# NVIDIA/cuopt

Measured on AMD Instinct MI355X. Metric: pdlp_iterations_per_sec, higher is better.
Workload: dtype f64; 1 GPU; c3: synthetic random sparse LP S(m=1000000,n=1000000,k=10,seed=2), nnz=10000000, longest row 10, CSR fp64/int32, Stable2 preset, tolerances 0 (fixed iteration budget); rows=1000000, cols=1000000, nnz=10000000, parallelism=single GPU

## Files before the change

### cuopt_amd/csrc/pdlp_epilogues.hpp

```cpp
#pragma once
#include "pdlp_kernels.hpp"

using namespace pdlp;

namespace p2pdev {
struct Peers {
  char* base[16];
};
constexpr int kKinds = 3;
__device__ __forceinline__ bool active(const pdlpdev_ctl* ctl) { return ctl->error == 0 && ctl->steps_taken < ctl->target_steps; }

struct Push {
  Peers P;
  int world, rank, kind;
  size_t dst_off, flag_off;
  unsigned long long* epoch;
  int lo[16], hi[16];
  __device__ __forceinline__ double* slot(int q) const { return reinterpret_cast<double*>(P.base[q] + dst_off); }
  __device__ __forceinline__ bool wants(int q, int i) const { return q != rank && i >= lo[q] && i < hi[q]; }
};
__device__ __forceinline__ void put(double* p, double v) { __hip_atomic_store(p, v, __ATOMIC_RELAXED, __HIP_MEMORY_SCOPE_SYSTEM); }
__device__ __forceinline__ void count_exchange(const Push* T)
{
  if (blockIdx.x == 0 && threadIdx.x == 0) T->epoch[T->kind] = T->epoch[T->kind] + 1;
}
__device__ __forceinline__ void raise(const Push* T)
{
  if (blockIdx.x != 0 || threadIdx.x != 0) return;
  const unsigned long long e = T->epoch[T->kind];
  for (int q = 0; q < T->world; ++q) {
    unsigned long long* flag = reinterpret_cast<unsigned long long*>(T->P.base[q] + T->flag_off) + (size_t)T->kind * T->world + T->rank;
    __hip_atomic_store(flag, e, __ATOMIC_RELEASE, __HIP_MEMORY_SCOPE_SYSTEM);
  }
}
__device__ __forceinline__ bool wait_flags(const unsigned long long* flags, int world, int kind, const unsigned long long* epoch)
{
  bool ok = true;
  if ((int)threadIdx.x < world) {
    const unsigned long long want = epoch[kind];
    const unsigned long long* f   = flags + (size_t)kind * world + threadIdx.x;
    const unsigned long long t0   = wall_clock64();
    while (__hip_atomic_load(f, __ATOMIC_RELAXED, __HIP_MEMORY_SCOPE_SYSTEM) < want) {
      __builtin_amdgcn_s_sleep(8);
      if (wall_clock64() - t0 > 500000000ull) {
        ok = false;
        break;
      }
    }
  }
  ok = __syncthreads_and(ok);
  if (threadIdx.x == 0) __threadfence_system();
  __syncthreads();
  return ok;
}
}


struct DualEpilogue {
  static constexpr int NQ = 1;
  using Op = SumOp;
  const double* __restrict__ y;
  double* __restrict__ yn;
  const double* __restrict__ lo;
  const double* __restrict__ hi;
  double* __restrict__ sumy;
  double sigma, weight;
  bool pend;
  double* __restrict__ copy = nullptr;
  const p2pdev::Push* __restrict__ push = nullptr;
  struct Ops {
    double y, lo, hi, sum;
  };
  __device__ __forceinline__ Ops load(int i) const { return Ops{y[i], lo[i], hi[i], pend ? sumy[i] : 0.0}; }
  __device__ __forceinline__ void apply(int i, double v, const Ops& o, double (&acc)[1])
  {
    const double yi = o.y;
    double next     = yi - (sigma * v);
    const double low = next + sigma * o.lo;
    const double up  = next + sigma * o.hi;
    next            = dmax(low, dmin(up, 0.0));
    yn[i]           = next;
    if (copy) copy[i] = next;
    if (push)
      for (int q = 0; q < push->world; ++q)
        if (push->wants(q, i)) p2pdev::put(push->slot(q) + i, next);
    const double dy = next - yi;
    acc[0] += dy * dy;
    if (pend) sumy[i] = o.sum + weight * yi;
  }
  __device__ __forceinline__ void row(int i, double v, double (&acc)[1]) { apply(i, v, load(i), acc); }
  static __device__ __forceinline__ DualEpilogue make(const pdlpdev_ctl* ctl, double* y0, double* y1, const double* lo, const double* hi,
                                                      double* sumy, double* ycopy, const p2pdev::Push* push)
  {
    const int cur = ctl->cur;
    return DualEpilogue{cur ? y1 : y0, cur ? y0 : y1, lo, hi, sumy, ctl->sigma, ctl->step_size, ctl->pending_avg != 0, ycopy, push};
  }
};

struct StepEpilogue {
  static constexpr int NQ = 2;
  using Op = SumOp;
  const double* __restrict__ x;
  const double* __restrict__ xn;
  const double* __restrict__ aty;
  double* __restrict__ atyn;
  struct Ops {
    double x, xn, aty;
  };
  __device__ __forceinline__ Ops load(int j) const { return Ops{x[j], xn[j], aty[j]}; }
  __device__ __forceinline__ void apply(int j, double v, const Ops& o, double (&acc)[2])
  {
    atyn[j]         = v;
    const double dx = o.xn - o.x;
    const double t  = v - o.aty;
    acc[0] += t * dx;
    acc[1] += dx * dx;
  }
  __device__ __forceinline__ void row(int j, double v, double (&acc)[2]) { apply(j, v, load(j), acc); }
  static __device__ __forceinline__ StepEpilogue make(const pdlpdev_ctl* ctl, const double* x0, const double* x1, double* aty0, double* aty1)
  {
    const int cur = ctl->cur;
    return StepEpilogue{cur ? x1 : x0, cur ? x0 : x1, cur ? aty1 : aty0, cur ? aty0 : aty1};
  }
};

struct HalpernWeights {
  double w, w0;
  __device__ __forceinline__ explicit HalpernWeights(const pdlpdev_halpern* hal)
  {
    const double k = (double)hal->k;
    w              = (k + 1.0) / (k + 2.0);
    w0             = 1.0 - w;
  }
  __device__ __forceinline__ double combine(double t, double z, double z0) const { return w * (2.0 * t - z) + w0 * z0; }
};
struct HalpernArgs {
  const pdlpdev_halpern* __restrict__ hal;
  double* __restrict__ tx;
  double* __restrict__ ty;
  const double* __restrict__ x0;
  const double* __restrict__ y0;
  const double* __restrict__ aty0;
};
__device__ __forceinline__ bool halpern_last_step(const pdlpdev_ctl* ctl) { return ctl->steps_taken + 1 >= ctl->target_steps; }
struct HalpernDualEpilogue {
  static constexpr int NQ = 1;
  using Op = SumOp;
  const double* __restrict__ y;
  double* __restrict__ yn;
  double* __restrict__ yp;
  const double* __restrict__ y0;
  const double* __restrict__ lo;
  const double* __restrict__ hi;
  double sigma;
  HalpernWeights hw;
  __device__ __forceinline__ void row(int i, double v, double (&acc)[1])
  {
    const double yi  = y[i];
    double next      = yi - (sigma * v);
    const double low = next + sigma * lo[i];
    const double up  = next + sigma * hi[i];
    next             = dmax(low, dmin(up, 0.0));
    yp[i]            = next;
    const double dy  = next - yi;
    acc[0] += dy * dy;
    yn[i] = hw.combine(next, yi, y0[i]);
  }
  static __device__ __forceinline__ HalpernDualEpilogue make(const pdlpdev_ctl* ctl, double* y0, double* y1, const double* lo, const double* hi,
                                                             const HalpernArgs& h)
  {
    const int cur = ctl->cur;
    return HalpernDualEpilogue{cur ? y1 : y0, cur ? y0 : y1, h.ty, h.y0, lo, hi, ctl->sigma, HalpernWeights(h.hal)};
  }
};
struct HalpernStepEpilogue {
  static constexpr int NQ = 2;
  using Op = SumOp;
  const double* __restrict__ x;
  double* __restrict__ xn;
  const double* __restrict__ aty;
  double* __restrict__ atyn;
  const double* __restrict__ x0;
  const double* __restrict__ aty0;
  double* __restrict__ xp;
  HalpernWeights hw;
  __device__ __forceinline__ void row(int j, double v, double (&acc)[2])
  {
    const double xj = x[j], xt = xn[j], a = aty[j];
    const double dx = xt - xj;
    const double t  = v - a;
    acc[0] += t * dx;
    acc[1] += dx * dx;
    if (xp) xp[j] = xt;
    xn[j]   = hw.combine(xt, xj, x0[j]);
    atyn[j] = hw.combine(v, a, aty0[j]);
  }
  static __device__ __forceinline__ HalpernStepEpilogue make(const pdlpdev_ctl* ctl, double* x0, double* x1, double* aty0, double* aty1,
                                                             const HalpernArgs& h)
  {
    const int cur = ctl->cur;
    return HalpernStepEpilogue{cur ? x1 : x0, cur ? x0 : x1, cur ? aty1 : aty0, cur ? aty0 : aty1, h.x0, h.aty0,
                               halpern_last_step(ctl) ? h.tx : nullptr, HalpernWeights(h.hal)};
  }
};

struct StoreEpilogue {
  static constexpr int NQ = 0;
  using Op = SumOp;
  double* __restrict__ out;
  __device__ __forceinline__ void row(int r, double v, double (&)[1]) { out[r] = v; }
  static __device__ __forceinline__ StoreEpilogue iterate(int side, double* aty0, double* aty1, double* out_override)
  {
    return StoreEpilogue{out_override ? out_override : (side ? aty1 : aty0)};
  }
};

__device__ __forceinline__ const double* evaluated(int cur, int which, const double* v0, const double* v1, const double* avg)
{
  return which == PDLPDEV_AVERAGE ? avg : (cur ? v1 : v0);
}

struct EvalPrimalEpilogue {
  static constexpr int NQ = 3;
  using Op = SumOp;
  const double* __restrict__ yhat;
  const double* __restrict__ dr;
  const double* __restrict__ lo_u;
  const double* __restrict__ hi_u;
  double eps_rel;
  double* __restrict__ linf_rows;
  double* __restrict__ ax_out;
  __device__ __forceinline__ void row(int i, double v, double (&acc)[3])
  {
    const double d  = dr[i];
    const double ax = v / d;
    ax_out[i]       = ax;
    const double yi = yhat[i] * d;
    const double lo = lo_u[i], hi = hi_u[i];
    const double rp = violation(ax, lo, hi);
    acc[0] += rp * rp;
    acc[1] += bound_value_product(yi, lo, hi);
    acc[2] += yi * yi;
    if (linf_rows) linf_rows[i] = rp - eps_rel * combine_bounds(lo, hi);
  }
};

struct EvalDualCore {
  const double* __restrict__ xhat;
  const double* __restrict__ dc;
  const double* __restrict__ c_u;
  const double* __restrict__ lb_u;
  const double* __restrict__ ub_u;
  double eps_rel;
  int rule_finite;
  double* __restrict__ rc_out;
  double* __restrict__ linf_rows;
  double* __restrict__ aty_out;
  __device__ __forceinline__ void col(int j, double aty_scaled, double (&acc)[4])
  {
    const double d    = dc[j];
    const double aty  = aty_scaled / d;
    aty_out[j]        = aty;
    const double cj   = c_u[j];
    const double g    = cj - aty;
    const double xj   = xhat[j] * d;
    const double lb   = lb_u[j], ub = ub_u[j];
    const double bv   = g > 0.0 ? lb : ub;
    double rc;
    if (g == 0.0)
      rc = g;
    else if (rule_finite)
      rc = dfinite(bv) ? g : 0.0;
    else
      rc = fabs(xj - bv) <= fabs(xj) ? g : 0.0;
    const double rd = g - rc;
    rc_out[j]       = rc;
    acc[0] += rd * rd;
    acc[1] += bound_value_product(rc, lb, ub);
    acc[2] += cj * xj;
    acc[3] += xj * xj;
    if (linf_rows) linf_rows[j] = rd - eps_rel * cj;
  }
};

struct EvalDualEpilogue {
  static constexpr int NQ = 4;
  using Op = SumOp;
  EvalDualCore core;
  __device__ __forceinline__ void row(int j, double v, double (&acc)[4]) { core.col(j, v, acc); }
};

struct DenseView {
  const int32_t* __restrict__ row;
  const int32_t* __restrict__ row_seg;
  const int32_t* __restrict__ seg_row;
  const int32_t* __restrict__ seg_c0;
  const int32_t* __restrict__ seg_len;
  const int32_t* __restrict__ seg_ptr;
  const int32_t* __restrict__ tile_ptr;
  const int32_t* __restrict__ tile_seg;
  const int32_t* __restrict__ tile_id;
  const double* __restrict__ val;
  const int32_t* __restrict__ ch_seg;
  const int32_t* __restrict__ ch_k0;
  const int32_t* __restrict__ row_ch;
  double* __restrict__ ch_part;
};

constexpr int kDenseChunk = 4096;

enum GatherMode : int {
  kGatherFixed   = 0,
  kGatherTrial   = 1,
  kGatherCurrent = 2,
};
static_assert(kGatherFixed == 0 && kGatherTrial == 1 && kGatherCurrent == 2, "the values of the kernels' `mode` argument");
__device__ __forceinline__ const double* pick_vector(const pdlpdev_ctl* ctl, const double* v0, const double* v1, int mode)
{
  if (mode == kGatherFixed) return v0;
  const bool cur = ctl->cur != 0;
  return (cur == (mode == kGatherTrial)) ? v0 : v1;
}
```

### cuopt_amd/csrc/spmv_panel.hpp

```cpp
#pragma once
#include "pdlp_kernels.hpp"

namespace pdlp {

struct PanelChunk {
  int s, c0, c1, t0;
  bool valid;
};
template <int R>
__device__ __forceinline__ void panel_load(const PanelView& P, double (&va)[kPanelPer], int (&ja)[kPanelPer], int c0, int c1)
{
#pragma unroll
  for (int u = 0; u < R; ++u) {
    int k = c0 + threadIdx.x + u * kPanelThreads;
    if (u == R - 1) k = k < c1 ? k : c1 - 1;
    va[u] = __builtin_nontemporal_load(P.val + k);
    ja[u] = __builtin_nontemporal_load(P.col + k);
  }
}
template <int R>
__device__ __forceinline__ void panel_products(const double* __restrict__ vec, double* prod, const double (&va)[kPanelPer],
                                               const int (&ja)[kPanelPer], int len)
{
  double x[R];
#pragma unroll
  for (int u = 0; u < R; ++u) x[u] = vec[ja[u]];
#pragma unroll
  for (int u = 0; u < R; ++u) {
    const int i = threadIdx.x + u * kPanelThreads;
    if (u < R - 1 || i < len) prod[i] = va[u] * x[u];
  }
}
#define PANEL_DISPATCH(rounds, CALL) \
  switch (rounds) {                   \
    case 1: CALL(1); break;           \
    case 2: CALL(2); break;           \
    case 3: CALL(3); break;           \
    case 4: CALL(4); break;           \
    case 5: CALL(5); break;           \
    case 6: CALL(6); break;           \
    case 7: CALL(7); break;           \
    default: CALL(8); break;          \
  }

template <class Epi>
__device__ __forceinline__ void panel_own_row(const PanelView& P, const double* __restrict__ vec, Epi& epi, double* __restrict__ partials,
                                              int w, int NP, double* scratch )
{
  const int r  = P.own_row[w - NP];
  const int k0 = P.csr_off[r], k1 = P.csr_off[r + 1];
  double part[1] = {0.0};
  constexpr int kLongU = 16;
  for (int k = k0 + (int)threadIdx.x; k < k1; k += kLongU * kPanelThreads) {
    double a[kLongU];
    int j[kLongU];
#pragma unroll
    for (int u = 0; u < kLongU; ++u) {
      a[u] = 0.0, j[u] = 0;
      if (k + u * kPanelThreads < k1) {
        a[u] = __builtin_nontemporal_load(P.csr_val + k + u * kPanelThreads);
        j[u] = __builtin_nontemporal_load(P.csr_idx + k + u * kPanelThreads);
      }
    }
    double xv[kLongU];
#pragma unroll
    for (int u = 0; u < kLongU; ++u) xv[u] = k + u * kPanelThreads < k1 ? vec[j[u]] : 0.0;
#pragma unroll
    for (int u = 0; u < kLongU; ++u) part[0] = part[0] + a[u] * xv[u];
  }
  if (P.dn_own_seg) {
    for (int sg = P.dn_own_seg[w - NP]; sg < P.dn_own_seg[w - NP + 1]; ++sg) {
      const int len = P.dn_seg_len[sg];
      const double* __restrict__ a = P.dn_val + P.dn_seg_ptr[sg];
      const double* __restrict__ x = vec + P.dn_seg_c0[sg];
      constexpr int kSegU = 8;
      for (int k = (int)threadIdx.x; k < len; k += kSegU * kPanelThreads) {
        double av[kSegU], xv[kSegU];
#pragma unroll
        for (int u = 0; u < kSegU; ++u) {
          const int i = k + u * kPanelThreads;
          av[u] = i < len ? __builtin_nontemporal_load(a + i) : 0.0;
          xv[u] = i < len ? x[i] : 0.0;
        }
#pragma unroll
        for (int u = 0; u < kSegU; ++u) part[0] = part[0] + av[u] * xv[u];
      }
    }
  }
  block_reduce<SumOp, 1, kPanelWaves>(part, scratch);
  double acc[Epi::NQ > 0 ? Epi::NQ : 1];
#pragma unroll
  for (int q = 0; q < (Epi::NQ > 0 ? Epi::NQ : 1); ++q) acc[q] = Epi::Op::identity();
  if (threadIdx.x == 0) {
    epi.row(r, dense_plus(P.dense_add, r, part[0]), acc);
    if constexpr (Epi::NQ > 0) {
#pragma unroll
      for (int q = 0; q < Epi::NQ; ++q) partials[(size_t)q * P.W + w] = acc[q];
    }
  }
}
struct PanelDenseSegs {
  int n;
  int c0[kPanelDenseSegs], len[kPanelDenseSegs], ptr[kPanelDenseSegs];
  double y[kPanelDenseSegs];
};
__device__ __forceinline__ void panel_dense_prepare(const PanelView& P, int w, const double* __restrict__ vec, PanelDenseSegs* D)
{
  if (!P.dn_pan_ptr) return;
  const int q0 = P.dn_pan_ptr[w], n = P.dn_pan_ptr[w + 1] - q0;
  if (threadIdx.x == 0) D->n = n;
  if ((int)threadIdx.x < n) {
    const int sg = P.dn_pan_seg[q0 + threadIdx.x];
    D->c0[threadIdx.x] = P.dn_seg_c0[sg], D->len[threadIdx.x] = P.dn_seg_len[sg], D->ptr[threadIdx.x] = P.dn_seg_ptr[sg];
    D->y[threadIdx.x]  = vec[P.dn_seg_row[sg]];
  }
}
__device__ __forceinline__ double panel_dense_col(const PanelView& P, const PanelDenseSegs* D, int j)
{
  double add   = 0.0;
  const int ns = D->n;
  for (int q = 0; q < ns; ++q) {
    const int k = j - D->c0[q];
    if (k >= 0 && k < D->len[q]) add += __builtin_nontemporal_load(P.dn_val + D->ptr[q] + k) * D->y[q];
  }
  return add;
}
template <class Epi>
__device__ __forceinline__ void panel_epilogue(const PanelView& P, Epi& epi, double* __restrict__ partials, const double* psum, double* red,
                                               int w, int r0, int nr, const PanelDenseSegs* D,
                                               const double* psum2 = nullptr )
{
  double acc[Epi::NQ > 0 ? Epi::NQ : 1];
#pragma unroll
  for (int q = 0; q < (Epi::NQ > 0 ? Epi::NQ : 1); ++q) acc[q] = Epi::Op::identity();
  for (int r = threadIdx.x; r < nr; r += kPanelThreads)
    if (__double_as_longlong(psum[r]) != kPanelNotMine) {
      double v = psum2 ? psum[r] + psum2[r] : psum[r];
      if (P.dn_pan_ptr) v = v + panel_dense_col(P, D, r0 + r);
      epi.row(r0 + r, dense_plus(P.dense_add, r0 + r, v), acc);
    }
  if constexpr (Epi::NQ > 0) {
    block_reduce<typename Epi::Op, Epi::NQ, kPanelWaves>(acc, red);
    if (threadIdx.x == 0) {
#pragma unroll
      for (int q = 0; q < Epi::NQ; ++q) partials[(size_t)q * P.W + w] = acc[q];
    }
  }
}

template <class Epi>
__device__ __forceinline__ void panel_spmv_block(const PanelView& P, const double* __restrict__ vec,
                                                 Epi& epi, double* __restrict__ partials)
{
  static_assert(kPanelPer == 8, "PANEL_DISPATCH enumerates 1..8 rounds");
  __shared__ double prod[kPanelChunk];
  __shared__ double psum[kPanelMaxRows];
  __shared__ double red[kPanelWaves * (Epi::NQ > 0 ? Epi::NQ : 1)];
  __shared__ int tile_s[17];
  __shared__ long long base_s[16];
  const int w  = blockIdx.x;
  const int NP = P.NP ? P.NP : P.W;
  if (w >= NP) {
    panel_own_row(P, vec, epi, partials, w, NP, prod);
    return;
  }
  __shared__ PanelDenseSegs dseg;
  const int r0 = P.row0[w], nr = P.row0[w + 1] - r0;
  panel_dense_prepare(P, w, vec, &dseg);
  if (threadIdx.x <= P.S) tile_s[threadIdx.x] = P.tile_ptr[w * P.S + threadIdx.x];
  if (threadIdx.x < P.S) base_s[threadIdx.x] = P.rp_base[w * P.S + threadIdx.x];
  for (int r = threadIdx.x; r < nr; r += kPanelThreads) psum[r] = 0.0;
  __syncthreads();
  if (P.own_ptr)
    for (int q = P.own_ptr[w] + (int)threadIdx.x; q < P.own_ptr[w + 1]; q += kPanelThreads) psum[P.own_row[q] - r0] = __longlong_as_double(kPanelNotMine);
  auto advance = [&](PanelChunk c) -> PanelChunk {
    if (c.valid && c.c1 < tile_s[c.s + 1]) {
      c.c0 = c.c1;
      c.c1 = c.c0 + kPanelChunk < tile_s[c.s + 1] ? c.c0 + kPanelChunk : tile_s[c.s + 1];
      return c;
    }
    int s = c.s + 1;
    while (s < P.S && tile_s[s + 1] == tile_s[s]) ++s;
    c.valid = s < P.S;
    c.s     = s;
    if (c.valid) {
      c.t0 = c.c0 = tile_s[s];
      c.c1 = c.c0 + kPanelChunk < tile_s[s + 1] ? c.c0 + kPanelChunk : tile_s[s + 1];
    }
    return c;
  };
  double va[kPanelPer];
  int ja[kPanelPer];
  unsigned ext_next[kPanelRowsPer], ext[kPanelRowsPer];
#define PANEL_ROUNDS(c) (((c).c1 - (c).c0 + kPanelThreads - 1) / kPanelThreads)
#define PANEL_CALL_LOAD(R) panel_load<R>(P, va, ja, nxt.c0, nxt.c1)
#define PANEL_CALL_PRODUCTS(R) panel_products<R>(vec, prod, va, ja, cur.c1 - cur.c0)
#define PANEL_REQUEST(c)                                                         \
  if ((c).valid) {                                                               \
    PANEL_DISPATCH(PANEL_ROUNDS(c), PANEL_CALL_LOAD)                             \
    const uint16_t* __restrict__ rp_ = P.rowptr + base_s[(c).s];                 \
    _Pragma("unroll") for (int q = 0; q < kPanelRowsPer; ++q) {                  \
      int r_      = threadIdx.x + q * kPanelThreads;                             \
      r_          = r_ < nr ? r_ : 0;                                            \
      ext_next[q] = (unsigned)rp_[r_] | ((unsigned)rp_[r_ + 1] << 16);           \
    }                                                                            \
  }
  PanelChunk none{-1, 0, 0, 0, false};
  PanelChunk nxt = advance(none);
  PANEL_REQUEST(nxt)
  PanelChunk cur = nxt;
  while (cur.valid) {
    __syncthreads();
    PANEL_DISPATCH(PANEL_ROUNDS(cur), PANEL_CALL_PRODUCTS)
#pragma unroll
    for (int q = 0; q < kPanelRowsPer; ++q) ext[q] = ext_next[q];
    const int lo = cur.c0 - cur.t0, hi = cur.c1 - cur.t0;
    nxt = advance(cur);
    PANEL_REQUEST(nxt)
    __syncthreads();
    if (!P.any_long) {
#pragma unroll
      for (int q = 0; q < kPanelRowsPer; ++q) {
        const int r = threadIdx.x + q * kPanelThreads;
        if (r < nr) {
          int a = (int)(ext[q] & 0xFFFFu), b = (int)(ext[q] >> 16);
          a = a > lo ? a : lo;
          b = b < hi ? b : hi;
          if (a < b) {
            double sum = psum[r];
            for (int k = a; k < b; ++k) sum = sum + prod[k - lo];
            psum[r] = sum;
          }
        }
      }
      cur = nxt;
      continue;
    }
    bool any_long = false;
#pragma unroll
    for (int q = 0; q < kPanelRowsPer; ++q) {
      const int r = threadIdx.x + q * kPanelThreads;
      if (r < nr) {
        int a = (int)(ext[q] & 0xFFFFu), b = (int)(ext[q] >> 16);
        a = a > lo ? a : lo;
        b = b < hi ? b : hi;
        if (b - a > kLongRow) {
          any_long = true;
        } else if (a < b) {
          double sum = psum[r];
          for (int k = a; k < b; ++k) sum = sum + prod[k - lo];
          psum[r] = sum;
        }
      }
    }
    if (__ballot(any_long)) {
#pragma unroll
      for (int q = 0; q < kPanelRowsPer; ++q) {
        const int r = threadIdx.x + q * kPanelThreads;
        int a = 0, b = 0;
        if (r < nr) {
          a = (int)(ext[q] & 0xFFFFu), b = (int)(ext[q] >> 16);
          a = a > lo ? a : lo;
          b = b < hi ? b : hi;
        }
        unsigned long long todo = __ballot(b - a > kLongRow);
        while (todo) {
          const int l  = __builtin_ctzll(todo);
          todo &= todo - 1;
          const int la = __builtin_amdgcn_readlane(a, l), lb = __builtin_amdgcn_readlane(b, l);
          double part  = 0.0;
          for (int k = la + (int)(threadIdx.x & 63); k < lb; k += 64) part = part + prod[k - lo];
          part = wave_reduce<SumOp>(part);
          if ((int)(threadIdx.x & 63) == l) psum[r] = psum[r] + part;
        }
      }
    }
    cur = nxt;
  }
#undef PANEL_REQUEST
#undef PANEL_CALL_PRODUCTS
#undef PANEL_CALL_LOAD
#undef PANEL_ROUNDS
  __syncthreads();
  panel_epilogue(P, epi, partials, psum, red, w, r0, nr, &dseg);
}
template <int CTRL, int ROW_MASK>
__device__ __forceinline__ double seg_dpp(double v)
{
  int lo = __double2loint(v), hi = __double2hiint(v);
  lo = __builtin_amdgcn_update_dpp(0, lo, CTRL, ROW_MASK, 0xf, false);
  hi = __builtin_amdgcn_update_dpp(0, hi, CTRL, ROW_MASK, 0xf, false);
  return __hiloint2double(hi, lo);
}
__device__ __forceinline__ double seg_scan(double S, int lane, int seg0)
{
  double u;
  u = seg_dpp<0x111, 0xf>(S); if ((lane & 15) >= 1 && lane - 1 >= seg0) S = S + u;
  u = seg_dpp<0x112, 0xf>(S); if ((lane & 15) >= 2 && lane - 2 >= seg0) S = S + u;
  u = seg_dpp<0x114, 0xf>(S); if ((lane & 15) >= 4 && lane - 4 >= seg0) S = S + u;
  u = seg_dpp<0x118, 0xf>(S); if ((lane & 15) >= 8 && lane - 8 >= seg0) S = S + u;
  u = seg_dpp<0x142, 0xa>(S); if ((lane & 16) && (lane | 15) - 16 >= seg0) S = S + u;
  u = seg_dpp<0x143, 0xc>(S); if (lane >= 32 && 31 >= seg0) S = S + u;
  return S;
}
__device__ __forceinline__ void seg_emit(double* strip, int row, double v)
{
  __hip_atomic_fetch_add(strip + row, v, __ATOMIC_RELAXED, __HIP_MEMORY_SCOPE_WORKGROUP);
}
struct SegRecord {
  double lsum, rsum;
  int lkey, rkey;
};
template <int R>
__device__ __forceinline__ void seg_load(const PanelView& P, double (&va)[kPanelPer], int (&pk)[kPanelPer], int c0, int c1)
{
#pragma unroll
  for (int u = 0; u < R; ++u) {
    int k = c0 + threadIdx.x + u * kPanelThreads;
    if (u == R - 1) k = k < c1 ? k : c1 - 1;
    va[u] = __builtin_nontemporal_load(P.val + k);
    pk[u] = __builtin_nontemporal_load(P.col + k);
  }
}
template <int R>
__device__ __forceinline__ void seg_rounds(const double* __restrict__ vec, int slab_base, const double (&va)[kPanelPer], const int (&pk)[kPanelPer], int len,
                                           double* psum, SegRecord* rec , int lane)
{
  double x[R];
#pragma unroll
  for (int u = 0; u < R; ++u) x[u] = vec[slab_base + (int)((unsigned)pk[u] & kSegColMask)];
#pragma unroll
  for (int u = 0; u < R; ++u) {
    const int i   = threadIdx.x + u * kPanelThreads;
    const int key = (int)((unsigned)pk[u] >> kSegColBits);
    const double v = (u < R - 1 || i < len) ? va[u] * x[u] : 0.0;
    const int prev = __builtin_amdgcn_update_dpp(-1, key, 0x138, 0xf, 0xf, false);
    const unsigned long long starts = __ballot(key != prev);
    const unsigned long long below  = starts & ((2ull << lane) - 1ull);
    const int seg0                  = 63 - __builtin_clzll(below);
    const double S                  = seg_scan(v, lane, seg0);
    const bool ends                 = lane == 63 || ((starts >> (lane + 1)) & 1ull);
    if (ends) {
      if (seg0 == 0) {
        rec[u].lsum = S, rec[u].lkey = key;
        if (lane == 63) rec[u].rkey = -1;
      } else if (lane == 63) {
        rec[u].rsum = S, rec[u].rkey = key;
      } else {
        seg_emit(psum, key, S);
      }
    }
  }
}
template <class Epi>
__device__ __forceinline__ void panel_seg_block(const PanelView& P, const double* __restrict__ vec, Epi& epi, double* __restrict__ partials)
{
  static_assert(kPanelPer == 8 && kPanelWaves == 8, "64 wave-rounds per chunk: one lane of wave 0 each");
  static_assert(kPanelMaxRows <= (1 << (32 - kSegColBits)), "row within the panel must fit beside the column");
  __shared__ double psum[kPanelMaxRows];
  __shared__ double psum2[kPanelMaxRows];
  __shared__ double red[kPanelWaves * (Epi::NQ > 0 ? Epi::NQ : 1)];
  __shared__ SegRecord rec[2][kPanelWaves * kPanelPer];
  __shared__ int tile_s[17];
  const int w  = blockIdx.x;
  const int NP = P.NP ? P.NP : P.W;
  if (w >= NP) {
    panel_own_row(P, vec, epi, partials, w, NP, psum);
    return;
  }
  __shared__ PanelDenseSegs dseg;
  const int r0 = P.row0[w], nr = P.row0[w + 1] - r0;
  panel_dense_prepare(P, w, vec, &dseg);
  if (threadIdx.x <= P.S) tile_s[threadIdx.x] = P.tile_ptr[w * P.S + threadIdx.x];
  for (int r = threadIdx.x; r < nr; r += kPanelThreads) psum[r] = 0.0, psum2[r] = 0.0;
  __syncthreads();
  if (P.own_ptr)
    for (int q = P.own_ptr[w] + (int)threadIdx.x; q < P.own_ptr[w + 1]; q += kPanelThreads) psum[P.own_row[q] - r0] = __longlong_as_double(kPanelNotMine);
  auto advance = [&](PanelChunk c) -> PanelChunk {
    if (c.valid && c.c1 < tile_s[c.s + 1]) {
      c.c0 = c.c1;
      c.c1 = c.c0 + kPanelChunk < tile_s[c.s + 1] ? c.c0 + kPanelChunk : tile_s[c.s + 1];
      return c;
    }
    int s = c.s + 1;
    while (s < P.S && tile_s[s + 1] == tile_s[s]) ++s;
    c.valid = s < P.S;
    c.s     = s;
    if (c.valid) {
      c.t0 = c.c0 = tile_s[s];
      c.c1 = c.c0 + kPanelChunk < tile_s[s + 1] ? c.c0 + kPanelChunk : tile_s[s + 1];
    }
    return c;
  };
  const int lane = threadIdx.x & 63;
  const int wave = __builtin_amdgcn_readfirstlane(threadIdx.x >> 6);
  double va[kPanelPer];
  int pk[kPanelPer];
#define SEG_ROUNDS(c) (((c).c1 - (c).c0 + kPanelThreads - 1) / kPanelThreads)
#define SEG_CALL_LOAD(R) seg_load<R>(P, va, pk, nxt.c0, nxt.c1)
#define SEG_CALL_ROUNDS(R) seg_rounds<R>(vec, cur.s * P.slab_w, va, pk, cur.c1 - cur.c0, psum, &rec[parity][wave * kPanelPer], lane)
  PanelChunk none{-1, 0, 0, 0, false};
  PanelChunk nxt = advance(none);
  if (nxt.valid) { PANEL_DISPATCH(SEG_ROUNDS(nxt), SEG_CALL_LOAD) }
  PanelChunk cur = nxt;
  int parity = 0;
  while (cur.valid) {
    const int R = SEG_ROUNDS(cur);
    PANEL_DISPATCH(R, SEG_CALL_ROUNDS)
    nxt = advance(cur);
    if (nxt.valid) { PANEL_DISPATCH(SEG_ROUNDS(nxt), SEG_CALL_LOAD) }
    __syncthreads();
    if (wave == 0) {
      const int u = lane >> 3, q = lane & 7;
      const bool on = u < R;
      SegRecord g{0.0, 0.0, 0, -1};
      if (on) g = rec[parity][q * kPanelPer + u];
      const bool single = g.rkey < 0;
      const int my_first = g.lkey, my_last = single ? g.lkey : g.rkey;
      const double open  = on ? (single ? g.lsum : g.rsum) : 0.0;
      int prev_last      = __builtin_amdgcn_update_dpp(0, my_last, 0x138, 0xf, 0xf, false);
      if (lane == 0) prev_last = my_first;
      const bool flag = on && (!single || my_first != prev_last);
      const unsigned long long fm = __ballot(flag);
      const unsigned long long at_or_below = fm & ((2ull << lane) - 1ull);
      const int seg0  = at_or_below ? 63 - __builtin_clzll(at_or_below) : 0;
      const double S  = seg_scan(open, lane, seg0);
      double carry_in = seg_dpp<0x138, 0xf>(S);
      if (lane == 0) carry_in = 0.0;
      if (on) {
        int key    = prev_last;
        double sum = carry_in;
        if (my_first != key) {
          seg_emit(psum2, key, sum);
          key = my_first, sum = 0.0;
        }
        sum = sum + g.lsum;
        if (!single) {
          seg_emit(psum2, key, sum);
          key = g.rkey, sum = g.rsum;
        }
        if (lane == R * kPanelWaves - 1) seg_emit(psum2, key, sum);
      }
    }
    parity ^= 1;
    cur = nxt;
  }
#undef SEG_CALL_ROUNDS
#undef SEG_CALL_LOAD
#undef SEG_ROUNDS
  __syncthreads();
  panel_epilogue(P, epi, partials, psum, red, w, r0, nr, &dseg, psum2);
}
#undef PANEL_DISPATCH
template <bool SEG, class Epi>
__device__ __forceinline__ void panel_block(const PanelView& P, const double* __restrict__ vec, Epi& epi, double* __restrict__ partials)
{
  if constexpr (SEG) panel_seg_block(P, vec, epi, partials);
  else panel_spmv_block(P, vec, epi, partials);
}

}
```

Before: 6081 iterations/s.

## Prefetch epilogue operands before final panel chunk reduction in SpMV blocks

For Halpern epilogues that expose an Ops struct, the panel SpMV and segmented SpMV blocks now issue the epilogue's per-row global loads (y, lo, hi, y0 or x, xn, aty, x0, aty0) before finishing the last chunk's row sums or segment join. The loads then overlap with that final reduction and the barrier. Afterwards a waitcnt is issued and the prefetched values are applied for the first few row strides. Rows beyond the prefetch depth fall back to the original path. The change adds register pressure from holding four Ops records per thread, and the row-sum and segment-join code is moved into helper functions.

```diff
diff --git a/cuopt_amd/csrc/pdlp_epilogues.hpp b/cuopt_amd/csrc/pdlp_epilogues.hpp
--- a/cuopt_amd/csrc/pdlp_epilogues.hpp
+++ b/cuopt_amd/csrc/pdlp_epilogues.hpp
@@ -154,6 +154,22 @@
   const double* __restrict__ hi;
   double sigma;
   HalpernWeights hw;
+  struct Ops {
+    double y, lo, hi, y0;
+  };
+  __device__ __forceinline__ Ops load(int i) const { return Ops{y[i], lo[i], hi[i], y0[i]}; }
+  __device__ __forceinline__ void apply(int i, double v, const Ops& o, double (&acc)[1])
+  {
+    const double yi  = o.y;
+    double next      = yi - (sigma * v);
+    const double low = next + sigma * o.lo;
+    const double up  = next + sigma * o.hi;
+    next             = dmax(low, dmin(up, 0.0));
+    yp[i]            = next;
+    const double dy  = next - yi;
+    acc[0] += dy * dy;
+    yn[i] = hw.combine(next, yi, o.y0);
+  }
   __device__ __forceinline__ void row(int i, double v, double (&acc)[1])
   {
     const double yi  = y[i];
@@ -184,6 +200,21 @@
   const double* __restrict__ aty0;
   double* __restrict__ xp;
   HalpernWeights hw;
+  struct Ops {
+    double x, xn, aty, x0, aty0;
+  };
+  __device__ __forceinline__ Ops load(int j) const { return Ops{x[j], xn[j], aty[j], x0[j], aty0[j]}; }
+  __device__ __forceinline__ void apply(int j, double v, const Ops& o, double (&acc)[2])
+  {
+    const double xj = o.x, xt = o.xn, a = o.aty;
+    const double dx = xt - xj;
+    const double t  = v - a;
+    acc[0] += t * dx;
+    acc[1] += dx * dx;
+    if (xp) xp[j] = xt;
+    xn[j]   = hw.combine(xt, xj, o.x0);
+    atyn[j] = hw.combine(v, a, o.aty0);
+  }
   __device__ __forceinline__ void row(int j, double v, double (&acc)[2])
   {
     const double xj = x[j], xt = xn[j], a = aty[j];
diff --git a/cuopt_amd/csrc/spmv_panel.hpp b/cuopt_amd/csrc/spmv_panel.hpp
--- a/cuopt_amd/csrc/spmv_panel.hpp
+++ b/cuopt_amd/csrc/spmv_panel.hpp
@@ -1,4 +1,6 @@
 #pragma once
+#include <type_traits>
+
 #include "pdlp_kernels.hpp"
 
 namespace pdlp {
@@ -126,24 +128,140 @@
   return add;
 }
 template <class Epi>
-__device__ __forceinline__ void panel_epilogue(const PanelView& P, Epi& epi, double* __restrict__ partials, const double* psum, double* red,
-                                               int w, int r0, int nr, const PanelDenseSegs* D,
-                                               const double* psum2 = nullptr )
-{
-  double acc[Epi::NQ > 0 ? Epi::NQ : 1];
-#pragma unroll
-  for (int q = 0; q < (Epi::NQ > 0 ? Epi::NQ : 1); ++q) acc[q] = Epi::Op::identity();
-  for (int r = threadIdx.x; r < nr; r += kPanelThreads)
+__device__ __forceinline__ void panel_epilogue_rows(const PanelView& P, Epi& epi, double (&acc)[Epi::NQ > 0 ? Epi::NQ : 1], const double* psum,
+                                                    int first, int r0, int nr, const PanelDenseSegs* D, const double* psum2)
+{
+  for (int r = first; r < nr; r += kPanelThreads)
     if (__double_as_longlong(psum[r]) != kPanelNotMine) {
       double v = psum2 ? psum[r] + psum2[r] : psum[r];
       if (P.dn_pan_ptr) v = v + panel_dense_col(P, D, r0 + r);
       epi.row(r0 + r, dense_plus(P.dense_add, r0 + r, v), acc);
     }
+}
+template <class Epi>
+__device__ __forceinline__ void panel_epilogue_partials(const PanelView& P, double* __restrict__ partials, double (&acc)[Epi::NQ > 0 ? Epi::NQ : 1],
+                                                        double* red, int w)
+{
   if constexpr (Epi::NQ > 0) {
     block_reduce<typename Epi::Op, Epi::NQ, kPanelWaves>(acc, red);
     if (threadIdx.x == 0) {
 #pragma unroll
       for (int q = 0; q < Epi::NQ; ++q) partials[(size_t)q * P.W + w] = acc[q];
+    }
+  }
+}
+template <class Epi>
+__device__ __forceinline__ void panel_epilogue(const PanelView& P, Epi& epi, double* __restrict__ partials, const double* psum, double* red,
+                                               int w, int r0, int nr, const PanelDenseSegs* D,
+                                               const double* psum2 = nullptr )
+{
+  double acc[Epi::NQ > 0 ? Epi::NQ : 1];
+#pragma unroll
+  for (int q = 0; q < (Epi::NQ > 0 ? Epi::NQ : 1); ++q) acc[q] = Epi::Op::identity();
+  panel_epilogue_rows(P, epi, acc, psum, threadIdx.x, r0, nr, D, psum2);
+  panel_epilogue_partials<Epi>(P, partials, acc, red, w);
+}
+
+constexpr int kPanelEpiDepth = 4;
+template <class Epi, class = void>
+struct PanelEarlyOps {
+  static constexpr bool on = false;
+  struct type {};
+};
+template <class Epi>
+struct PanelEarlyOps<Epi, std::void_t<typename Epi::Ops>> {
+  static constexpr bool on = true;
+  using type = typename Epi::Ops;
+};
+template <class Epi>
+__device__ __forceinline__ void panel_epilogue_request(const Epi& epi, typename Epi::Ops (&pre)[kPanelEpiDepth], int r0, int nr)
+{
+#pragma unroll
+  for (int q = 0; q < kPanelEpiDepth; ++q) {
+    int r  = threadIdx.x + q * kPanelThreads;
+    r      = r < nr ? r : 0;
+    pre[q] = epi.load(r0 + r);
+  }
+}
+template <class Epi>
+__device__ __forceinline__ void panel_epilogue_early(const PanelView& P, Epi& epi, double* __restrict__ partials, const double* psum, double* red,
+                                                     int w, int r0, int nr, const PanelDenseSegs* D,
+                                                     const typename Epi::Ops (&pre)[kPanelEpiDepth], const double* psum2 = nullptr)
+{
+  double acc[Epi::NQ > 0 ? Epi::NQ : 1];
+#pragma unroll
+  for (int q = 0; q < (Epi::NQ > 0 ? Epi::NQ : 1); ++q) acc[q] = Epi::Op::identity();
+  __builtin_amdgcn_s_waitcnt(0x0F70);
+#pragma unroll
+  for (int q = 0; q < kPanelEpiDepth; ++q) {
+    const int r = threadIdx.x + q * kPanelThreads;
+    if (r < nr && __double_as_longlong(psum[r]) != kPanelNotMine) {
+      double v = psum2 ? psum[r] + psum2[r] : psum[r];
+      if (P.dn_pan_ptr) v = v + panel_dense_col(P, D, r0 + r);
+      epi.apply(r0 + r, dense_plus(P.dense_add, r0 + r, v), pre[q], acc);
+    }
+  }
+  panel_epilogue_rows(P, epi, acc, psum, threadIdx.x + kPanelEpiDepth * kPanelThreads, r0, nr, D, psum2);
+  panel_epilogue_partials<Epi>(P, partials, acc, red, w);
+}
+
+__device__ __forceinline__ void panel_row_sums(const PanelView& P, const unsigned (&ext)[kPanelRowsPer], const double* prod, double* psum,
+                                               int nr, int lo, int hi)
+{
+  if (!P.any_long) {
+#pragma unroll
+    for (int q = 0; q < kPanelRowsPer; ++q) {
+      const int r = threadIdx.x + q * kPanelThreads;
+      if (r < nr) {
+        int a = (int)(ext[q] & 0xFFFFu), b = (int)(ext[q] >> 16);
+        a = a > lo ? a : lo;
+        b = b < hi ? b : hi;
+        if (a < b) {
+          double sum = psum[r];
+          for (int k = a; k < b; ++k) sum = sum + prod[k - lo];
+          psum[r] = sum;
+        }
+      }
+    }
+    return;
+  }
+  bool any_long = false;
+#pragma unroll
+  for (int q = 0; q < kPanelRowsPer; ++q) {
+    const int r = threadIdx.x + q * kPanelThreads;
+    if (r < nr) {
+      int a = (int)(ext[q] & 0xFFFFu), b = (int)(ext[q] >> 16);
+      a = a > lo ? a : lo;
+      b = b < hi ? b : hi;
+      if (b - a > kLongRow) {
+        any_long = true;
+      } else if (a < b) {
+        double sum = psum[r];
+        for (int k = a; k < b; ++k) sum = sum + prod[k - lo];
+        psum[r] = sum;
+      }
+    }
+  }
+  if (__ballot(any_long)) {
+#pragma unroll
+    for (int q = 0; q < kPanelRowsPer; ++q) {
+      const int r = threadIdx.x + q * kPanelThreads;
+      int a = 0, b = 0;
+      if (r < nr) {
+        a = (int)(ext[q] & 0xFFFFu), b = (int)(ext[q] >> 16);
+        a = a > lo ? a : lo;
+        b = b < hi ? b : hi;
+      }
+      unsigned long long todo = __ballot(b - a > kLongRow);
+      while (todo) {
+        const int l  = __builtin_ctzll(todo);
+        todo &= todo - 1;
+        const int la = __builtin_amdgcn_readlane(a, l), lb = __builtin_amdgcn_readlane(b, l);
+        double part  = 0.0;
+        for (int k = la + (int)(threadIdx.x & 63); k < lb; k += 64) part = part + prod[k - lo];
+        part = wave_reduce<SumOp>(part);
+        if ((int)(threadIdx.x & 63) == l) psum[r] = psum[r] + part;
+      }
     }
   }
 }
@@ -209,6 +327,9 @@
   PanelChunk nxt = advance(none);
   PANEL_REQUEST(nxt)
   PanelChunk cur = nxt;
+  constexpr bool kEarly = PanelEarlyOps<Epi>::on;
+  [[maybe_unused]] typename PanelEarlyOps<Epi>::type pre[kPanelEpiDepth];
+  [[maybe_unused]] int lo_last = 0, hi_last = 0;
   while (cur.valid) {
     __syncthreads();
     PANEL_DISPATCH(PANEL_ROUNDS(cur), PANEL_CALL_PRODUCTS)
@@ -216,73 +337,32 @@
     for (int q = 0; q < kPanelRowsPer; ++q) ext[q] = ext_next[q];
     const int lo = cur.c0 - cur.t0, hi = cur.c1 - cur.t0;
     nxt = advance(cur);
+    if constexpr (kEarly)
+      if (!nxt.valid) {
+        lo_last = lo, hi_last = hi;
+        break;
+      }
     PANEL_REQUEST(nxt)
     __syncthreads();
-    if (!P.any_long) {
-#pragma unroll
-      for (int q = 0; q < kPanelRowsPer; ++q) {
-        const int r = threadIdx.x + q * kPanelThreads;
-        if (r < nr) {
-          int a = (int)(ext[q] & 0xFFFFu), b = (int)(ext[q] >> 16);
-          a = a > lo ? a : lo;
-          b = b < hi ? b : hi;
-          if (a < b) {
-            double sum = psum[r];
-            for (int k = a; k < b; ++k) sum = sum + prod[k - lo];
-            psum[r] = sum;
-          }
-        }
-      }
-      cur = nxt;
-      continue;
-    }
-    bool any_long = false;
-#pragma unroll
-    for (int q = 0; q < kPanelRowsPer; ++q) {
-      const int r = threadIdx.x + q * kPanelThreads;
-      if (r < nr) {
-        int a = (int)(ext[q] & 0xFFFFu), b = (int)(ext[q] >> 16);
-        a = a > lo ? a : lo;
-        b = b < hi ? b : hi;
-        if (b - a > kLongRow) {
-          any_long = true;
-        } else if (a < b) {
-          double sum = psum[r];
-          for (int k = a; k < b; ++k) sum = sum + prod[k - lo];
-          psum[r] = sum;
-        }
-      }
-    }
-    if (__ballot(any_long)) {
-#pragma unroll
-      for (int q = 0; q < kPanelRowsPer; ++q) {
-        const int r = threadIdx.x + q * kPanelThreads;
-        int a = 0, b = 0;
-        if (r < nr) {
-          a = (int)(ext[q] & 0xFFFFu), b = (int)(ext[q] >> 16);
-          a = a > lo ? a : lo;
-          b = b < hi ? b : hi;
-        }
-        unsigned long long todo = __ballot(b - a > kLongRow);
-        while (todo) {
-          const int l  = __builtin_ctzll(todo);
-          todo &= todo - 1;
-          const int la = __builtin_amdgcn_readlane(a, l), lb = __builtin_amdgcn_readlane(b, l);
-          double part  = 0.0;
-          for (int k = la + (int)(threadIdx.x & 63); k < lb; k += 64) part = part + prod[k - lo];
-          part = wave_reduce<SumOp>(part);
-          if ((int)(threadIdx.x & 63) == l) psum[r] = psum[r] + part;
-        }
-      }
-    }
+    panel_row_sums(P, ext, prod, psum, nr, lo, hi);
     cur = nxt;
   }
 #undef PANEL_REQUEST
 #undef PANEL_CALL_PRODUCTS
 #undef PANEL_CALL_LOAD
 #undef PANEL_ROUNDS
-  __syncthreads();
-  panel_epilogue(P, epi, partials, psum, red, w, r0, nr, &dseg);
+  if constexpr (kEarly) {
+    panel_epilogue_request(epi, pre, r0, nr);
+    if (cur.valid) {
+      __syncthreads();
+      panel_row_sums(P, ext, prod, psum, nr, lo_last, hi_last);
+    }
+    __syncthreads();
+    panel_epilogue_early(P, epi, partials, psum, red, w, r0, nr, &dseg, pre);
+  } else {
+    __syncthreads();
+    panel_epilogue(P, epi, partials, psum, red, w, r0, nr, &dseg);
+  }
 }
 template <int CTRL, int ROW_MASK>
 __device__ __forceinline__ double seg_dpp(double v)
@@ -352,6 +432,39 @@
     }
   }
 }
+__device__ __forceinline__ void panel_seg_join(const SegRecord* rec , double* psum2, int R, int lane)
+{
+  const int u = lane >> 3, q = lane & 7;
+  const bool on = u < R;
+  SegRecord g{0.0, 0.0, 0, -1};
+  if (on) g = rec[q * kPanelPer + u];
+  const bool single = g.rkey < 0;
+  const int my_first = g.lkey, my_last = single ? g.lkey : g.rkey;
+  const double open  = on ? (single ? g.lsum : g.rsum) : 0.0;
+  int prev_last      = __builtin_amdgcn_update_dpp(0, my_last, 0x138, 0xf, 0xf, false);
+  if (lane == 0) prev_last = my_first;
+  const bool flag = on && (!single || my_first != prev_last);
+  const unsigned long long fm = __ballot(flag);
+  const unsigned long long at_or_below = fm & ((2ull << lane) - 1ull);
+  const int seg0  = at_or_below ? 63 - __builtin_clzll(at_or_below) : 0;
+  const double S  = seg_scan(open, lane, seg0);
+  double carry_in = seg_dpp<0x138, 0xf>(S);
+  if (lane == 0) carry_in = 0.0;
+  if (on) {
+    int key    = prev_last;
+    double sum = carry_in;
+    if (my_first != key) {
+      seg_emit(psum2, key, sum);
+      key = my_first, sum = 0.0;
+    }
+    sum = sum + g.lsum;
+    if (!single) {
+      seg_emit(psum2, key, sum);
+      key = g.rkey, sum = g.rsum;
+    }
+    if (lane == R * kPanelWaves - 1) seg_emit(psum2, key, sum);
+  }
+}
 template <class Epi>
 __device__ __forceinline__ void panel_seg_block(const PanelView& P, const double* __restrict__ vec, Epi& epi, double* __restrict__ partials)
 {
@@ -404,52 +517,39 @@
   if (nxt.valid) { PANEL_DISPATCH(SEG_ROUNDS(nxt), SEG_CALL_LOAD) }
   PanelChunk cur = nxt;
   int parity = 0;
+  constexpr bool kEarly = PanelEarlyOps<Epi>::on;
+  [[maybe_unused]] typename PanelEarlyOps<Epi>::type pre[kPanelEpiDepth];
+  [[maybe_unused]] int R_last = 0;
   while (cur.valid) {
     const int R = SEG_ROUNDS(cur);
     PANEL_DISPATCH(R, SEG_CALL_ROUNDS)
     nxt = advance(cur);
+    if constexpr (kEarly)
+      if (!nxt.valid) {
+        R_last = R;
+        break;
+      }
     if (nxt.valid) { PANEL_DISPATCH(SEG_ROUNDS(nxt), SEG_CALL_LOAD) }
     __syncthreads();
-    if (wave == 0) {
-      const int u = lane >> 3, q = lane & 7;
-      const bool on = u < R;
-      SegRecord g{0.0, 0.0, 0, -1};
-      if (on) g = rec[parity][q * kPanelPer + u];
-      const bool single = g.rkey < 0;
-      const int my_first = g.lkey, my_last = single ? g.lkey : g.rkey;
-      const double open  = on ? (single ? g.lsum : g.rsum) : 0.0;
-      int prev_last      = __builtin_amdgcn_update_dpp(0, my_last, 0x138, 0xf, 0xf, false);
-      if (lane == 0) prev_last = my_first;
-      const bool flag = on && (!single || my_first != prev_last);
-      const unsigned long long fm = __ballot(flag);
-      const unsigned long long at_or_below = fm & ((2ull << lane) - 1ull);
-      const int seg0  = at_or_below ? 63 - __builtin_clzll(at_or_below) : 0;
-      const double S  = seg_scan(open, lane, seg0);
-      double carry_in = seg_dpp<0x138, 0xf>(S);
-      if (lane == 0) carry_in = 0.0;
-      if (on) {
-        int key    = prev_last;
-        double sum = carry_in;
-        if (my_first != key) {
-          seg_emit(psum2, key, sum);
-          key = my_first, sum = 0.0;
-        }
-        sum = sum + g.lsum;
-        if (!single) {
-          seg_emit(psum2, key, sum);
-          key = g.rkey, sum = g.rsum;
-        }
-        if (lane == R * kPanelWaves - 1) seg_emit(psum2, key, sum);
-      }
-    }
+    if (wave == 0) panel_seg_join(rec[parity], psum2, R, lane);
     parity ^= 1;
     cur = nxt;
   }
 #undef SEG_CALL_ROUNDS
 #undef SEG_CALL_LOAD
 #undef SEG_ROUNDS
-  __syncthreads();
-  panel_epilogue(P, epi, partials, psum, red, w, r0, nr, &dseg, psum2);
+  if constexpr (kEarly) {
+    panel_epilogue_request(epi, pre, r0, nr);
+    if (cur.valid) {
+      __syncthreads();
+      if (wave == 0) panel_seg_join(rec[parity], psum2, R_last, lane);
+    }
+    __syncthreads();
+    panel_epilogue_early(P, epi, partials, psum, red, w, r0, nr, &dseg, pre, psum2);
+  } else {
+    __syncthreads();
+    panel_epilogue(P, epi, partials, psum, red, w, r0, nr, &dseg, psum2);
+  }
 }
 #undef PANEL_DISPATCH
 template <bool SEG, class Epi>
```

Measured after the change: 6258 iterations/s, median of 6. 1.03x the previous value.
